# qiyunzhu/woltka

Measured on AMD Instinct MI355X. Metric: alignment records/sec classified, higher is better.
Workload: dtype u8; 1 GPU; synthetic SAM text of 50M reads x <=16 hits (10.50 GB) resident in HBM, 2M-node taxonomy, ranks phylum,genus,species: device tokenizer per 64 MB block + one weighted histogram per sample (the kernels of `woltka classify`, host link left out); records_per_gpu=250034804, reads_per_gpu=50000000

## Files before the change

woltka_amd/csrc/wk_dtok_fused.hpp:

```cpp
#pragma once
#include "wk_dtok.hpp"
#include "wk_dtok_neighbour.hpp"
#include "wk_dtok_planes.hpp"
#include "wk_dtok_rounds.hpp"

namespace wk {

constexpr uint32_t kFzThreads = 512;
constexpr uint32_t kFzWaves = kFzThreads / kWave;
constexpr uint32_t kFzTile = 16384;
constexpr uint32_t kFzBack = 1024;
constexpr uint32_t kFzFwd = 3072;
constexpr uint32_t kFzWin = kFzTile + kFzBack + kFzFwd;
constexpr uint32_t kFzChunks = kFzWin / 16 + 1;
constexpr uint32_t kFzRounds = kFrMaxRounds;
static_assert(kFrChunks * 16u == kFzWin && kFrTailChunk + 1u == kFzChunks && kFrWaves == kFzWaves && kFrWave == kWave,
              "the dealing covers the window");
constexpr uint32_t kFzLines = 1024;
constexpr uint32_t kFzStreams = 4;
constexpr uint32_t kFzCap = 1024;
static_assert(kFzCap >= kFzLines, "a window's records fit an empty buffer");
static_assert(kFzWin + 32 < 65536, "window offsets fit 16 bits");
constexpr uint32_t kFzCarry = 256;
static_assert(kFzCarry + kFzLines <= kFpMaxLines && kFzThreads % kWave == 0, "a window's owned lines fit the planes, a wave's lines one word");

constexpr uint32_t kDtokSpill = 64;

struct FusedArgs {
    const unsigned char* text;
    uint32_t n;
    uint32_t open_end;
    uint32_t span;
    const struct DictSlot8* dict8;
    const uint4* names16;
    uint32_t dict_mask;
    const unsigned char* arena;
    uint2* unknown;
    uint32_t unknown_cap;
    DtokState* state;
    DtokState* host_state;
    const unsigned long long* backup_prev;
    unsigned long long* backup_next;
    uint32_t* host_seq;
    uint32_t seq;
    StreamSet streams;
    const int32_t* submap;
    uint32_t n_submap;
    uint32_t ablate;
};

static_assert(sizeof(DtokState) % 8 == 0, "the packed totals are aligned");
__device__ __forceinline__ unsigned long long* fz_totals(DtokState* state) { return reinterpret_cast<unsigned long long*>(state + 1); }

__global__ void dtok_fused_begin_kernel(unsigned long long* __restrict__ backup, const unsigned long long* __restrict__ cursor, DtokState* state) {
    if (threadIdx.x < (uint32_t)kMaxStreams) backup[threadIdx.x] = cursor[threadIdx.x];
    if (threadIdx.x == 0) {
        *state = DtokState{0u, 0u, 0ull, 0ull, 0ull, 0u, 0u};
        *fz_totals(state) = 0ull;
    }
}

template <int kCtrl, int kRowMask>
__device__ __forceinline__ uint32_t fz_dpp_add(uint32_t v) {
    return v + (uint32_t)__builtin_amdgcn_update_dpp(0, (int)v, kCtrl, kRowMask, 0xF, false);
}
__device__ __forceinline__ uint32_t fz_wave_scan(uint32_t v) {
    static_assert(kWave == 64, "four rows of sixteen lanes");
    v = fz_dpp_add<0x111, 0xF>(v);
    v = fz_dpp_add<0x112, 0xF>(v);
    v = fz_dpp_add<0x114, 0xF>(v);
    v = fz_dpp_add<0x118, 0xF>(v);
    v = fz_dpp_add<0x142, 0xA>(v);
    v = fz_dpp_add<0x143, 0xC>(v);
    return v;
}
__device__ __forceinline__ uint32_t fz_last_lane(uint32_t v) { return (uint32_t)__builtin_amdgcn_readlane((int)v, kWave - 1); }
__device__ __forceinline__ uint32_t fz_wave_sum(uint32_t v) { return fz_last_lane(fz_wave_scan(v)); }
__device__ __forceinline__ unsigned long long fz_first_lane64(unsigned long long v) {
    return ((unsigned long long)(uint32_t)__builtin_amdgcn_readfirstlane((int)(uint32_t)(v >> 32)) << 32) |
           (uint32_t)__builtin_amdgcn_readfirstlane((int)(uint32_t)v);
}

__device__ __forceinline__ uint4 fz_load_stream(const unsigned char* p) {
    typedef uint32_t u32x4 __attribute__((ext_vector_type(4)));
    const u32x4 v = __builtin_nontemporal_load(reinterpret_cast<const u32x4*>(p));
    return make_uint4(v.x, v.y, v.z, v.w);
}
__device__ __forceinline__ unsigned long long fz_load64(const unsigned char* p) {
    unsigned long long w;
    __builtin_memcpy(&w, p, 8);
    return w;
}
__device__ __forceinline__ uint32_t fz_load32(const unsigned char* p) {
    uint32_t w;
    __builtin_memcpy(&w, p, 4);
    return w;
}
__device__ __forceinline__ unsigned long long fz_eq_bytes(unsigned long long w, unsigned char c) {
    const unsigned long long x = w ^ (0x0101010101010101ull * c);
    return ~(((x & 0x7F7F7F7F7F7F7F7Full) + 0x7F7F7F7F7F7F7F7Full) | x | 0x7F7F7F7F7F7F7F7Full);
}
__device__ __forceinline__ uint32_t fz_marks32(uint32_t w, uint32_t c4) {
    const uint32_t x = w ^ c4;
    return ~(((x & 0x7F7F7F7Fu) + 0x7F7F7F7Fu) | x | 0x7F7F7F7Fu);
}
__device__ __forceinline__ unsigned long long fz_low_bytes(unsigned long long w, uint32_t k) {
    return k >= 8u ? w : (w & ((1ull << (8u * k)) - 1ull));
}

__device__ __forceinline__ unsigned long long fz_hash(const unsigned char* p, uint32_t n) {
    unsigned long long h = 0xcbf29ce484222325ull ^ ((unsigned long long)n * 0x9E3779B97F4A7C15ull);
    while (n >= 8u) {
        h = (h ^ fz_load64(p)) * 0x100000001b3ull;
        h ^= h >> 29;
        p += 8;
        n -= 8u;
    }
    const unsigned long long v = n ? fz_low_bytes(fz_load64(p), n) : 0ull;
    h = (h ^ v) * 0x100000001b3ull;
    h ^= h >> 32;
    h *= 0x9E3779B97F4A7C15ull;
    return h ^ (h >> 29);
}

__device__ __forceinline__ bool fz_same(const unsigned char* x, const unsigned char* y, uint32_t n) {
    while (n >= 8u) {
        if (fz_load64(x) != fz_load64(y)) return false;
        x += 8;
        y += 8;
        n -= 8u;
    }
    return n == 0u || fz_low_bytes(fz_load64(x) ^ fz_load64(y), n) == 0ull;
}

struct FzProbe {
    unsigned long long hv, n0, n1;
    uint32_t h;
    uint2 slot;
};
__device__ __forceinline__ FzProbe fz_probe_begin(const FusedArgs& a, const unsigned char* name, uint32_t rn) {
    FzProbe p;
    p.n0 = p.n1 = 0ull;
    if (rn <= 15u) {
        const unsigned long long lo = fz_low_bytes(fz_load64(name), rn), hi = rn > 8u ? fz_low_bytes(fz_load64(name + 8), rn - 8u) : 0ull;
        p.n0 = lo;
        p.n1 = hi | ((unsigned long long)rn << 56);
        unsigned long long h = 0xcbf29ce484222325ull ^ ((unsigned long long)rn * 0x9E3779B97F4A7C15ull), v = lo;
        if (rn >= 8u) {
            h = (h ^ lo) * 0x100000001b3ull;
            h ^= h >> 29;
            v = hi;
        }
        h = (h ^ v) * 0x100000001b3ull;
        h ^= h >> 32;
        h *= 0x9E3779B97F4A7C15ull;
        p.hv = h ^ (h >> 29);
    } else {
        p.hv = fz_hash(name, rn);
    }
    p.h = (uint32_t)p.hv & a.dict_mask;
    p.slot = reinterpret_cast<const uint2*>(a.dict8)[p.h];
    return p;
}
__device__ __forceinline__ int32_t fz_probe_end(const FusedArgs& a, FzProbe p, const unsigned char* name, uint32_t rn, uint32_t abs_off) {
    for (;;) {
        const int32_t id = (int32_t)p.slot.y;
        if (id < 0) break;
        if (p.slot.x == (uint32_t)(p.hv >> 32)) {
            const uint4 nm = a.names16[id];
            const unsigned long long s0 = ((unsigned long long)nm.y << 32) | nm.x, s1 = ((unsigned long long)nm.w << 32) | nm.z;
            if (rn <= 15u) {
                if (s0 == p.n0 && s1 == p.n1) return id;
            } else if ((nm.w >> 24) == 0xFFu) {
                const unsigned char* full = a.arena + nm.x;
                if (fz_load32(full) == rn && fz_same(name, full + 4, rn)) return id;
            }
        }
        p.h = (p.h + 1u) & a.dict_mask;
        p.slot = reinterpret_cast<const uint2*>(a.dict8)[p.h];
    }
    const uint32_t at = atomicAdd(&a.state->n_unknown, 1u);
    if (at < a.unknown_cap)
        a.unknown[at] = make_uint2(abs_off, rn);
    else
        atomicOr(&a.state->flags, kDtokUnknownFull);
    return kLineUnknown;
}

__device__ bool fz_starts_run_slow(const unsigned char* __restrict__ text, uint32_t at, const unsigned char* q, uint32_t qn) {
    uint32_t pos = at;
    while (pos > 0u) {
        const uint32_t e = pos - 1u;
        uint32_t s = e;
        while (s > 0u && text[s - 1u] != '\n') --s;
        uint32_t tab[3], nt = 0;
        for (uint32_t p = s; p < e && nt < 3u; ++p)
            if (text[p] == '\t') tab[nt++] = p;
        if (nt == 3u && !(tab[2] - tab[1] == 2u && text[tab[1] + 1u] == '*')) {
            if (tab[0] - s != qn) return true;
            for (uint32_t k = 0; k < qn; ++k)
                if (text[s + k] != q[k]) return true;
            return false;
        }
        pos = s;
    }
    return true;
}

constexpr uint32_t kFiSubj = (1u << 23) - 1u;
constexpr uint32_t kFiMateShift = 24;
constexpr uint32_t kFiMapped = 1u << 26;
constexpr uint32_t kFiStart = 1u << 27;
constexpr uint32_t kFiUndecided = 1u << 28;
constexpr uint32_t kFiExcl = 1u << 29;
constexpr uint32_t kFiDropped = 1u << 30;
constexpr uint32_t kFiRead = kFiMapped | (3u << kFiMateShift);
constexpr uint32_t kFiKey = kFiRead | kFiSubj;
constexpr uint32_t kFzPad = 8;
constexpr uint32_t kFzEdgeMeta = 4;

__device__ __forceinline__ uint32_t fz_octet(uint32_t z_lo, uint32_t z_hi) { return (((z_lo >> 7) | (z_hi >> 3)) * 0x00204081u >> 21) & 255u; }

__device__ __forceinline__ uint32_t fz_newlines16(uint4 v) {
    return fz_octet(fz_marks32(v.x, 0x0A0A0A0Au), fz_marks32(v.y, 0x0A0A0A0Au)) | (fz_octet(fz_marks32(v.z, 0x0A0A0A0Au), fz_marks32(v.w, 0x0A0A0A0Au)) << 8);
}

__device__ __forceinline__ uint32_t fz_tabs32(const unsigned char* p, unsigned long long* q0 = nullptr, unsigned long long* q1 = nullptr) {
    unsigned long long w[4];
#pragma unroll
    for (uint32_t i = 0; i < 4; ++i) w[i] = fz_load64(p + 8u * i);
    uint32_t m = 0;
#pragma unroll
    for (uint32_t i = 0; i < 4; ++i)
        m |= fz_octet(fz_marks32((uint32_t)w[i], 0x09090909u), fz_marks32((uint32_t)(w[i] >> 32), 0x09090909u)) << (8u * i);
    if (q0) {
        *q0 = w[0];
        *q1 = w[1];
    }
    return m;
}

__global__ void __launch_bounds__(kFzThreads) __attribute__((amdgpu_waves_per_eu(6, 6))) dtok_fused_kernel(FusedArgs a) {
    __shared__ __attribute__((aligned(16))) unsigned char txt[kFzChunks * 16 + 32];
    __shared__ uint16_t ls[kFzLines + 2];
    __shared__ uint16_t f_qn[kFzLines];
    __shared__ __attribute__((aligned(16))) uint32_t edge[kFzLines / kWave + 1][2][8];
    __shared__ __attribute__((aligned(16))) uint32_t info_[kFzPad + kFzCarry + kFzLines + kFzPad + 8];
    __shared__ uint32_t carry[kFzCarry];
    __shared__ unsigned long long planes[kFpPlanes][kFpWords];
    __shared__ uint32_t rbuf[kFzStreams][kFzCap];
    __shared__ unsigned long long fill_packed;
    static_assert(kFzStreams <= 4 && kFzCap + kFzThreads < 65536, "four 16-bit counts");
    __shared__ unsigned long long gbase[kFzStreams];
    __shared__ uint32_t wtot[kFzWaves];
    __shared__ unsigned long long gbase_out[kMaxStreams];
    __shared__ unsigned long long wg_totals;
    __shared__ uint32_t own[4];
    __shared__ uint32_t wg_flags;
    uint32_t* const info = info_ + kFzPad + kFzCarry;

    const uint32_t tid = threadIdx.x, lane = tid & (kWave - 1), wave = tid / kWave;
    const uint32_t wave_s = (uint32_t)__builtin_amdgcn_readfirstlane((int)wave);
    const uint32_t n_streams = a.streams.n_streams;
    const uint32_t ablate = a.ablate;
    const int32_t* const submap = a.submap;
    unsigned long long fill = 0ull;
    if (tid == 0) fill_packed = 0ull;
    if (tid < 4u) reinterpret_cast<uint32_t*>(txt + kFrTailChunk * 16u)[tid] = 0u;
    if (tid == 0) wg_flags = 0u;
    if (tid == 0) wg_totals = 0ull;
    if (tid == 0) edge[0][1][kFzEdgeMeta] = 0u;
    uint32_t my_flags = 0, my_reads = 0, my_lines = 0;
    const uint32_t text_end = a.n + (a.open_end ? 1u : 0u);

    auto flush_all = [&](unsigned long long have, bool last) {
        __syncthreads();
        if (tid < n_streams) {
            const uint32_t cnt = (ablate & 64u) ? 0u : (uint32_t)(have >> (16u * tid)) & 0xFFFFu;
            unsigned long long base = 0ull;
            if (cnt) {
                base = atomicAdd(&a.streams.cursor[tid], (unsigned long long)cnt);
                if (base + cnt > a.streams.cap) atomicOr(&wg_flags, kDtokSpill);
            }
            gbase[tid] = base;
        }
        __syncthreads();
        for (uint32_t k = 0; k < n_streams; ++k) {
            const uint32_t cnt = (ablate & 64u) ? 0u : (uint32_t)(have >> (16u * k)) & 0xFFFFu;
            const unsigned long long base = gbase[k];
            for (uint32_t i = tid; i < cnt; i += kFzThreads)
                if (base + i < a.streams.cap) a.streams.out[k][base + i] = rbuf[k][i];
        }
        if (last) return;
        __syncthreads();
    };

    const uint32_t t0 = blockIdx.x * a.span;
    const uint32_t t1 = a.n - t0 > a.span ? t0 + a.span : a.n;
    const uint32_t span_w1 = (uint32_t)min((unsigned long long)t1 + kFzFwd, (unsigned long long)text_end);
    uint32_t wpos = t0 >= kFzBack ? t0 - kFzBack : 0u;
    uint32_t mode = 0u;
    uint32_t counted = t0;
    bool wide = false;
    uint32_t nc = 0u;
    uint32_t cq_pos = 0u, cq_len = 0u;
    const uint32_t max_trips = a.span / 16u + 2u;
    for (uint32_t trip = 0;; ++trip) {
        if (trip >= max_trips) {
            my_flags |= kDtokSpill;
            break;
        }
        const uint32_t w0 = wpos & ~15u;
        const uint32_t lead = wpos - w0;
        const uint32_t w1 = (uint32_t)min((mode == 0u ? (unsigned long long)t0 + kFzTile + kFzFwd : (unsigned long long)w0 + kFzWin),
                                           (unsigned long long)(wide ? text_end : span_w1));
        const bool to_end = w1 == text_end;
        const bool last_win = wide || w1 == span_w1;
        __syncthreads();
        if (tid < 3u) own[tid] = tid < 2u ? 0xFFFFFFFFu : 0u;
        if (tid < kFzPad) info[-(int32_t)nc - 1 - (int32_t)tid] = kFiStart;
        for (uint32_t i = tid; i < nc; i += kFzThreads) info[(int32_t)i - (int32_t)nc] = carry[i];

        const uint32_t wave_c0 = fr_first_chunk(wave_s), wave_rounds = fr_rounds(wave_s);
        uint4 v[kFzRounds];
#pragma unroll
        for (uint32_t r = 0; r < kFzRounds; ++r) {
            const uint32_t p = w0 + (wave_c0 + r * kWave + lane) * 16u;
            v[r] = make_uint4(0u, 0u, 0u, 0u);
            if (r < wave_rounds && p < a.n && p < w1) v[r] = fz_load_stream(a.text + p);
        }
        uint32_t marks[kFzRounds];
        uint32_t nl_packed = 0;
        bool blank = false;
        const uint32_t in_lo = max(wpos, counted), in_hi = min(min(w1, a.n), t1);
#pragma unroll
        for (uint32_t r = 0; r < kFzRounds; ++r) {
            const uint32_t c = wave_c0 + r * kWave + lane;
            const uint32_t p = w0 + c * 16u;
            marks[r] = 0u;
            if (r >= wave_rounds) continue;
            const uint32_t rp0 = w0 + (wave_c0 + r * kWave) * 16u;
            const bool interior = rp0 >= in_lo && (unsigned long long)rp0 + kWave * 16u <= in_hi;
            *reinterpret_cast<uint4*>(txt + c * 16u) = v[r];
            if (interior) {
                const uint32_t m = fr_chunk_marks(fz_newlines16(v[r]), &blank);
                const uint32_t cnt = (uint32_t)__popc(m);
                my_lines += cnt;
                marks[r] = m;
                nl_packed |= fr_pack(cnt, r);
            } else if (p < w1) {
                uint32_t m = fz_newlines16(v[r]);
                if (p + 16u > a.n) m &= p >= a.n ? 0u : (1u << (a.n - p)) - 1u;
                if (p >= counted && p < t1) my_lines += (uint32_t)__popc(m);
                if (a.open_end && a.n >= p && a.n < p + 16u) m |= 1u << (a.n - p);
                if (p + 16u > w1) m &= (1u << (w1 - p)) - 1u;
                if (p < wpos) m &= ~((1u << (wpos - p)) - 1u);
                m = fr_chunk_marks(m, &blank);
                marks[r] = m;
                nl_packed |= fr_pack((uint32_t)__popc(m), r);
            }
        }
        if (blank && !(ablate & 16u)) my_flags |= kDtokShortLine;
        const uint32_t nl_inc = fz_wave_scan(nl_packed);
        const uint32_t nl_wave = fz_last_lane(nl_inc);
        if (lane == 0) wtot[wave] = fr_total(nl_wave);
        __syncthreads();
        uint32_t before = 0, total_nl = 0;
#pragma unroll
        for (uint32_t w = 0; w < kFzWaves; ++w) {
            before += w < wave ? wtot[w] : 0u;
            total_nl += wtot[w];
        }
        const bool too_many = total_nl + 1u > kFzLines || (ablate & (32u | 512u));
        if (too_many) {
            if (!(ablate & 512u)) my_flags |= kDtokSpill;
        } else {
            if (tid == 0) ls[0] = (uint16_t)lead;
            uint32_t line = before;
#pragma unroll
            for (uint32_t r = 0; r < kFzRounds; ++r) {
                if (r >= wave_rounds) continue;
                const uint32_t c = wave_c0 + r * kWave + lane;
                uint32_t at = line + fr_unpack(nl_inc, r) - (uint32_t)__popc(marks[r]);
                uint32_t m = marks[r];
                while (m) {
                    const uint32_t b = (uint32_t)__ffs((int)m) - 1u;
                    ls[++at] = (uint16_t)(c * 16u + b + 1u);
                    m &= m - 1u;
                }
                line += fr_unpack(nl_wave, r);
            }
        }
        __syncthreads();
        const uint32_t trail = too_many ? wpos : w0 + (uint32_t)__builtin_amdgcn_readfirstlane((int)(uint32_t)ls[total_nl]);
        if (!too_many && last_win && trail >= t0 && trail < t1) my_flags |= kDtokSpill;
        const uint32_t first_line = mode != 0u || w0 == 0u ? 0u : 1u;
        const uint32_t n_lines = too_many ? 0u : total_nl;
        if (tid == 0 && first_line) info[0] = 0u;

        for (uint32_t k0 = first_line; k0 < n_lines; k0 += kFzThreads) {
            const uint32_t k = k0 + tid;
            const bool has = k < n_lines;
            uint32_t word = 0, s = 0, qn = 0, rb = 0, rn = 0;
            unsigned long long q0 = 0ull, q1 = 0ull;
            if (has) {
                s = ls[k];
                const uint32_t e = (uint32_t)ls[k + 1] - 1u;
                uint32_t tab[3] = {0, 0, 0}, nt = 0;
                if (!(ablate & 256u)) {
                    uint32_t m = fz_tabs32(txt + s, &q0, &q1);
                    if (e - s < 32u) m &= (1u << (e - s)) - 1u;
                    nt = min((uint32_t)__popc(m), 3u);
                    tab[0] = s + (uint32_t)__ffs((int)m) - 1u;
                    m &= m - 1u;
                    tab[1] = s + (uint32_t)__ffs((int)m) - 1u;
                    m &= m - 1u;
                    tab[2] = s + (uint32_t)__ffs((int)m) - 1u;
                    for (uint32_t p = s + 32u; nt < 3u && p < e; p += 32u) {
                        m = fz_tabs32(txt + p);
                        if (e - p < 32u) m &= (1u << (e - p)) - 1u;
                        for (; m && nt < 3u; m &= m - 1u) {
                            const uint32_t q = p + (uint32_t)__ffs((int)m) - 1u;
                            if (nt == 0u)
                                tab[0] = q;
                            else if (nt == 1u)
                                tab[1] = q;
                            else
                                tab[2] = q;
                            ++nt;
                        }
                    }
                }
                if (ablate & 16u) {
                } else if (nt < 3u) {
                    my_flags |= kDtokShortLine;
                } else {
                    const uint32_t fl = tab[1] - tab[0] - 1u;
                    const unsigned long long fw = fz_load64(txt + tab[0] + 1u);
                    uint32_t flag = 0;
                    bool digits = fl >= 1u && fl <= 6u;
                    for (uint32_t i = 0; i < fl && i < 6u; ++i) {
                        const uint32_t d = ((uint32_t)(fw >> (8u * i)) & 0xFFu) - (uint32_t)'0';
                        digits &= d <= 9u;
                        flag = flag * 10u + d;
                    }
                    rb = tab[1] + 1u;
                    rn = tab[2] - rb;
                    if (!digits) {
                        my_flags |= kDtokShortLine;
                    } else if (rn == 1u && txt[rb] == '*') {
                    } else {
                        const uint32_t mate = (flag >> 6) & 3u;
                        if (mate == 3u) my_flags |= kDtokBothMates;
                        word = kFiMapped | (mate << kFiMateShift);
                        qn = tab[0] - s;
                        f_qn[k] = (uint16_t)qn;
                    }
                }
            }
            const bool mapped = (word & kFiMapped) != 0u, look = mapped && w0 + s >= t0;
            const unsigned char* const name = txt + rb;
            FzProbe probe;
            if (look && !(ablate & 1u)) probe = fz_probe_begin(a, name, rn);
            const FnLine me = has ? fn_line(mapped, qn, q0, q1) : fn_no_line();
            FnLine prev;
            prev.meta = (uint32_t)__builtin_amdgcn_update_dpp(0, (int)me.meta, 0x138 , 0xF, 0xF, false);
#pragma unroll
            for (uint32_t i = 0; i < 4; ++i) prev.b[i] = (uint32_t)__builtin_amdgcn_update_dpp(0, (int)me.b[i], 0x138, 0xF, 0xF, false);
            const uint32_t verdict = (ablate & 8u) ? (uint32_t)kFnStarts : (uint32_t)fn_verdict(prev, me);
            if (lane == 0 || lane == kWave - 1u) {
                uint32_t* const to = lane == 0 ? edge[(k0 - first_line) / kWave + wave][0] : edge[(k0 - first_line) / kWave + wave + 1u][1];
                *reinterpret_cast<uint4*>(to) = make_uint4(me.b[0], me.b[1], me.b[2], me.b[3]);
                to[kFzEdgeMeta] = me.meta;
            }
            const bool start = look && verdict == kFnStarts;
            if (look) {
                int32_t sid = (ablate & 1u) ? (int32_t)(fz_load32(name + 4) % 1000u) : fz_probe_end(a, probe, name, rn, w0 + rb);
                bool excluded = false;
                if (submap && sid >= 0) {
                    if ((uint32_t)sid < a.n_submap) {
                        sid = submap[sid];
                        if (sid == kLineExcluded) {
                            excluded = true;
                            sid = 0;
                        }
                    } else {
                        my_flags |= kDtokSpill;
                        sid = -1;
                    }
                }
                word |= (start ? kFiStart : 0u) | (verdict == kFnUndecided ? kFiUndecided : 0u) | (excluded ? kFiExcl : 0u) |
                        (sid < 0 ? kFiSubj : ((uint32_t)sid & kFiSubj));
            }
            if (has) info[k] = word;
            const unsigned long long b_all = __ballot(start), b_in = __ballot(start && w0 + s < t1), b_out = b_all & ~b_in;
            if (lane == 0 && b_all) {
                if (b_in) atomicMin(&own[0], k + (uint32_t)__builtin_ctzll(b_in));
                if (b_out) atomicMin(&own[1], k + (uint32_t)__builtin_ctzll(b_out));
                atomicMax(&own[2], k + 63u - (uint32_t)__builtin_clzll(b_all));
            }
        }
        __syncthreads();
        for (uint32_t k0 = first_line; k0 < n_lines; k0 += kFzThreads) {
            const uint32_t k = k0 + tid;
            const uint32_t mk = k < n_lines ? info[k] : 0u;
            bool und = (mk & kFiUndecided) != 0u, start = false;
            if (lane == 0 && und) {
                const uint32_t g = (k0 - first_line) / kWave + wave;
                FnLine before, me;
#pragma unroll
                for (uint32_t i = 0; i < 4; ++i) {
                    before.b[i] = edge[g][1][i];
                    me.b[i] = edge[g][0][i];
                }
                before.meta = edge[g][1][kFzEdgeMeta];
                me.meta = edge[g][0][kFzEdgeMeta];
                const FnVerdict v = fn_verdict(before, me);
                und = v == kFnUndecided;
                start = v == kFnStarts;
                if (g == 0u && nc == 0u && (mode == 1u || wpos == 0u)) {
                    und = false;
                    start = true;
                }
            }
            if (__ballot(und) != 0ull) {
                if (und) {
                    uint32_t j = k;
                    bool found = false;
                    while (j > first_line) {
                        --j;
                        if (info[j] & kFiMapped) {
                            found = true;
                            break;
                        }
                    }
                    if (found)
                        start = f_qn[j] != f_qn[k] || !fz_same(txt + ls[k], txt + ls[j], f_qn[k]);
                    else if (nc)
                        start = f_qn[k] != cq_len || !fz_same(txt + ls[k], a.text + cq_pos, cq_len);
                    else if (mode == 1u || wpos == 0u)
                        start = true;
                    else
                        start = fz_starts_run_slow(a.text, w0 + ls[first_line], txt + ls[k], f_qn[k]);
                }
            }
            if (mk & kFiUndecided) {
                info[k] = (mk & ~kFiUndecided) | (start ? kFiStart : 0u);
                if (start) {
                    atomicMin(&own[w0 + ls[k] < t1 ? 0 : 1], k);
                    atomicMax(&own[2], k);
                }
            }
        }
        __syncthreads();
        const uint32_t o0 = (uint32_t)__builtin_amdgcn_readfirstlane((int)own[0]), o1 = (uint32_t)__builtin_amdgcn_readfirstlane((int)own[1]);
        const uint32_t last = (uint32_t)__builtin_amdgcn_readfirstlane((int)own[2]);
        const uint32_t lpos = w0 + (uint32_t)__builtin_amdgcn_readfirstlane((int)(uint32_t)ls[o0 != 0xFFFFFFFFu ? last : 0u]);
        const bool has_first = nc != 0u || o0 != 0xFFFFFFFFu;
        const int32_t first_own = nc ? -(int32_t)nc : (int32_t)o0;
        int32_t ka = 0, kb = 0;
        uint32_t next = 0u, next_mode = 0u, nc_next = 0u;
        bool more = false, again = false, put_aside = false;
        if (too_many) {
            if ((ablate & (32u | 512u)) && !last_win) {
                next = w1;
                next_mode = 2u;
                more = true;
            }
        } else if (o1 != 0xFFFFFFFFu) {
            kb = (int32_t)o1;
            ka = has_first ? first_own : kb;
        } else if (to_end) {
            kb = (int32_t)n_lines;
            ka = has_first ? first_own : kb;
        } else if (last_win && a.span <= kFzTile) {
            if (o0 != 0xFFFFFFFFu) my_flags |= kDtokSpill;
        } else if (o0 != 0xFFFFFFFFu && (nc != 0u || last != o0 || lpos > wpos)) {
            kb = (int32_t)last;
            ka = first_own;
            next = lpos;
            next_mode = 1u;
            more = true;
            again = last_win;
        } else if (o0 != 0xFFFFFFFFu && last_win && !wide) {
            next = wpos;
            next_mode = 1u;
            more = again = true;
        } else if (o0 != 0xFFFFFFFFu || nc != 0u) {
            put_aside = true;
        } else if (!last_win) {
            next = trail;
            next_mode = 2u;
            more = trail > wpos && trail < t1;
            if (trail <= wpos) my_flags |= kDtokSpill;
        }
        if (put_aside) {
            if (tid == 0) {
                uint32_t c = nc;
                for (uint32_t k = first_line; k < n_lines; ++k) {
                    const uint32_t w = info[k];
                    if (w & kFiMapped) {
                        if (c < kFzCarry) carry[c] = w & ~kFiDropped;
                        ++c;
                    }
                }
                own[3] = c;
            }
            __syncthreads();
            nc_next = (uint32_t)__builtin_amdgcn_readfirstlane((int)own[3]);
            if (nc_next > kFzCarry || trail <= wpos) {
                my_flags |= kDtokSpill;
                nc_next = 0u;
            } else {
                if (nc == 0u) {
                    cq_pos = wpos;
                    cq_len = (uint32_t)__builtin_amdgcn_readfirstlane((int)(uint32_t)f_qn[0]);
                }
                next = trail;
                next_mode = 2u;
                more = true;
                again = last_win;
            }
        }
        for (int32_t k0 = ka; k0 < kb; k0 += (int32_t)kFzThreads) {
            const int32_t k = k0 + (int32_t)tid;
            const uint32_t mk = k < kb ? info[k] : 0u;
            const bool mapped = (mk & kFiMapped) != 0u, excl = mapped && (mk & kFiExcl);
            if (excl) {
                int32_t j = k;
                while (!(info[j] & kFiStart)) --j;
                atomicOr(&info[j], kFiDropped);
            }
            bool dup = false;
            if (mapped && !excl && !(mk & kFiStart) && !(ablate & 2u)) {
                bool done = false;
                for (int32_t j = k; !done; j -= 8) {
                    uint32_t w[8];
#pragma unroll
                    for (uint32_t i = 0; i < 8; ++i) w[i] = info[j - 1 - (int32_t)i];
#pragma unroll
                    for (uint32_t i = 0; i < 8; ++i) {
                        dup |= !done && ((w[i] ^ mk) & kFiKey) == 0u;
                        done |= (w[i] & kFiStart) != 0u;
                    }
                }
            }
            const bool first = mapped && !excl && !dup;
            const uint32_t mate = (mk >> kFiMateShift) & 3u;
            const uint32_t wi = (uint32_t)__builtin_amdgcn_readfirstlane((int)((uint32_t)(k0 - ka) / kWave + wave));
            const bool put = lane == 0 && wi < kFpWords;
            const unsigned long long p_start = __ballot(mapped && (mk & kFiStart));
            if (put) planes[kFpStart][wi] = p_start;
#pragma unroll
            for (uint32_t m = 0; m < 4; ++m) {
                const unsigned long long p_first = __ballot(first && mate == m);
                if (put) planes[kFpFirst + m][wi] = p_first;
            }
        }
        __syncthreads();
        for (int32_t k0 = ka; k0 < kb; k0 += (int32_t)kFzThreads) {
            const int32_t k = k0 + (int32_t)tid;
            bool rec = false;
            uint32_t word = 0, sl = 0, at = 0;
            const uint32_t li = (uint32_t)(k - ka);
            const uint32_t mk = k < kb ? info[k] : 0u;
            const unsigned long long* const mine = planes[kFpFirst + ((mk >> kFiMateShift) & 3u)];
            if (k < kb && ((mine[li / 64u] >> (li % 64u)) & 1ull) && !(ablate & 4u)) {
                uint32_t pos = 0, size = 1;
                bool dropped = (mk & kFiStart) && (mk & kFiDropped);
                if (!(ablate & (2u | 128u))) {
                    const FpRead r = fp_read(planes[kFpStart], mine, li, (uint32_t)(kb - ka));
                    pos = r.pos;
                    size = r.size;
                    dropped = (info[ka + (int32_t)r.head] & kFiDropped) != 0u;
                }
                if (size > (uint32_t)WK_WEIGHT_MAX_K) my_flags |= kDtokBigRead;
                const uint32_t s = mk & kFiSubj;
                if (s != kFiSubj && !dropped) {
                    rec = true;
                    word = s | ((pos & 15u) << kWordSubjBits) | ((size & 31u) << kWordSizeShift);
                    sl = s / kSliceBins;
                    if (sl >= n_streams) sl = n_streams - 1u;
                    my_reads += pos == 0u ? 1u : 0u;
                }
            }
            {
                unsigned long long add = 0;
                uint32_t mine_before = 0;
                for (uint32_t s2 = 0; s2 < n_streams; ++s2) {
                    const unsigned long long m = __ballot(rec && sl == s2);
                    add |= (unsigned long long)__popcll(m) << (16u * s2);
                    if (rec && sl == s2) mine_before = (uint32_t)__popcll(m & ((1ull << lane) - 1ull));
                }
                if (add) {
                    unsigned long long base = 0;
                    if (lane == 0) base = atomicAdd(&fill_packed, add);
                    base = fz_first_lane64(base);
                    at = (uint32_t)(base >> (16u * sl)) & 0xFFFFu;
                    at += mine_before;
                }
            }
            __syncthreads();
            unsigned long long now = fz_first_lane64(fill_packed);
            static_assert(kFzCap + 0x7BFFu == 0x7FFFu && 2u * kFzCap + kFzThreads + 0x7BFFu < 0x10000u, "the full test");
            if ((now + 0x7BFF7BFF7BFF7BFFull) & 0x8000800080008000ull) {
                flush_all(fill, false);
                at -= (uint32_t)(fill >> (16u * sl)) & 0xFFFFu;
                now -= fill;
                if (tid == 0) fill_packed = now;
            }
            if (rec) rbuf[sl][at] = word;
            fill = now;
            if (k0 + (int32_t)kFzThreads < kb) __syncthreads();
        }
        if (!more) break;
        wpos = next;
        mode = next_mode;
        wide = again;
        nc = nc_next;
        counted = w1;
    }
    if (my_flags) atomicOr(&wg_flags, my_flags);
    {
        const uint32_t reads_w = fz_wave_sum(my_reads), lines_w = fz_wave_sum(my_lines);
        const unsigned long long t = ((unsigned long long)lines_w << 32) | reads_w;
        if (lane == 0 && t) atomicAdd(&wg_totals, t);
    }
    flush_all(fill, true);
    __syncthreads();
    if (tid == 0) {
        if (wg_totals) __hip_atomic_fetch_add(fz_totals(a.state), wg_totals, __ATOMIC_RELAXED, __HIP_MEMORY_SCOPE_AGENT);
        if (wg_flags) atomicOr(&a.state->flags, wg_flags);
        __threadfence();
        own[0] = atomicAdd(&a.state->done, 1u) == gridDim.x - 1u ? 1u : 0u;
    }
    __syncthreads();
    if (own[0]) {
        __threadfence();
        uint32_t xt = tid;
        asm volatile("" : "+v"(xt));
        if (xt < (uint32_t)kMaxStreams) {
            const unsigned long long cur = __hip_atomic_load(&a.streams.cursor[xt], __ATOMIC_RELAXED, __HIP_MEMORY_SCOPE_AGENT);
            a.backup_next[xt] = cur;
            gbase_out[xt] = xt < n_streams ? cur - a.backup_prev[xt] : 0ull;
        }
        __syncthreads();
        if (tid == 0) {
            DtokState st{};
            st.flags = __hip_atomic_load(&a.state->flags, __ATOMIC_RELAXED, __HIP_MEMORY_SCOPE_AGENT);
            st.n_unknown = __hip_atomic_load(&a.state->n_unknown, __ATOMIC_RELAXED, __HIP_MEMORY_SCOPE_AGENT);
            const unsigned long long totals = __hip_atomic_load(fz_totals(a.state), __ATOMIC_RELAXED, __HIP_MEMORY_SCOPE_AGENT);
            for (uint32_t k = 0; k < (uint32_t)kMaxStreams; ++k) st.n_out += gbase_out[k];
            st.n_reads = totals & 0xFFFFFFFFull;
            st.n_lines = totals >> 32;
            *a.host_state = st;
            *a.state = DtokState{0u, 0u, 0ull, 0ull, 0ull, 0u, 0u};
            *fz_totals(a.state) = 0ull;
            __threadfence_system();
            if (a.host_seq) __hip_atomic_store(a.host_seq, a.seq, __ATOMIC_RELEASE, __HIP_MEMORY_SCOPE_SYSTEM);
        }
    }
}

}
```

woltka_amd/csrc/wk_dtok_neighbour.hpp:

```cpp
#pragma once
#include <cstdint>

#if defined(__HIPCC__) || defined(__CUDACC__)
#define WK_FN_FN __host__ __device__ __forceinline__
#else
#define WK_FN_FN inline
#endif

namespace wk {

constexpr uint32_t kFnLine = 1u << 16;
constexpr uint32_t kFnMapped = 1u << 17;
constexpr uint32_t kFnQn = 0xFFFFu;
constexpr uint32_t kFnBytes = 16;

struct FnLine {
    uint32_t meta;
    uint32_t b[4];
};

enum FnVerdict : uint32_t { kFnStarts = 0, kFnContinues = 1, kFnUndecided = 2 };

WK_FN_FN unsigned long long fn_low_bytes(unsigned long long w, uint32_t k) { return k >= 8u ? w : (w & ((1ull << (8u * k)) - 1ull)); }

WK_FN_FN FnLine fn_line(bool mapped, uint32_t qn, unsigned long long w0, unsigned long long w1) {
    FnLine l;
    l.meta = kFnLine | (mapped ? kFnMapped : 0u) | (qn & kFnQn);
    const unsigned long long m0 = fn_low_bytes(w0, qn), m1 = qn > 8u ? fn_low_bytes(w1, qn - 8u) : 0ull;
    l.b[0] = (uint32_t)m0;
    l.b[1] = (uint32_t)(m0 >> 32);
    l.b[2] = (uint32_t)m1;
    l.b[3] = (uint32_t)(m1 >> 32);
    return l;
}
WK_FN_FN FnLine fn_no_line() { return FnLine{0u, {0u, 0u, 0u, 0u}}; }

WK_FN_FN FnVerdict fn_verdict(const FnLine& prev, const FnLine& cur) {
    if ((prev.meta & (kFnLine | kFnMapped)) != (kFnLine | kFnMapped)) return kFnUndecided;
    const uint32_t diff = ((prev.meta ^ cur.meta) & kFnQn) | (prev.b[0] ^ cur.b[0]) | (prev.b[1] ^ cur.b[1]) | (prev.b[2] ^ cur.b[2]) | (prev.b[3] ^ cur.b[3]);
    if (diff) return kFnStarts;
    return (cur.meta & kFnQn) <= kFnBytes ? kFnContinues : kFnUndecided;
}

}
```

Baseline: 16.23 billion records/s.

## Deal lines with a witness lane per wave to drop edge shared-memory pass

The line pass now gives each wave 63 owned lines plus one witness lane that re-parses the previous line, so the DPP neighbour comparison covers wave boundaries without the edge array in shared memory. The second pass that resolved undecided lines is skipped entirely unless some wave saw an undecided verdict, tracked with a shared flag. This removes LDS traffic and a resolution sweep in the common case. The cost is about 1/64 redundant parsing work and more loop trips per window.

```diff
diff --git a/woltka_amd/csrc/wk_dtok_fused.hpp b/woltka_amd/csrc/wk_dtok_fused.hpp
--- a/woltka_amd/csrc/wk_dtok_fused.hpp
+++ b/woltka_amd/csrc/wk_dtok_fused.hpp
@@ -217,7 +217,7 @@
 constexpr uint32_t kFiRead = kFiMapped | (3u << kFiMateShift);
 constexpr uint32_t kFiKey = kFiRead | kFiSubj;
 constexpr uint32_t kFzPad = 8;
-constexpr uint32_t kFzEdgeMeta = 4;
+static_assert(kFwWave == kWave && kFwWaves == kFzWaves, "the line pass's dealing is this workgroup's");
 
 __device__ __forceinline__ uint32_t fz_octet(uint32_t z_lo, uint32_t z_hi) { return (((z_lo >> 7) | (z_hi >> 3)) * 0x00204081u >> 21) & 255u; }
 
@@ -244,7 +244,6 @@
     __shared__ __attribute__((aligned(16))) unsigned char txt[kFzChunks * 16 + 32];
     __shared__ uint16_t ls[kFzLines + 2];
     __shared__ uint16_t f_qn[kFzLines];
-    __shared__ __attribute__((aligned(16))) uint32_t edge[kFzLines / kWave + 1][2][8];
     __shared__ __attribute__((aligned(16))) uint32_t info_[kFzPad + kFzCarry + kFzLines + kFzPad + 8];
     __shared__ uint32_t carry[kFzCarry];
     __shared__ unsigned long long planes[kFpPlanes][kFpWords];
@@ -255,7 +254,7 @@
     __shared__ uint32_t wtot[kFzWaves];
     __shared__ unsigned long long gbase_out[kMaxStreams];
     __shared__ unsigned long long wg_totals;
-    __shared__ uint32_t own[4];
+    __shared__ uint32_t own[5];
     __shared__ uint32_t wg_flags;
     uint32_t* const info = info_ + kFzPad + kFzCarry;
 
@@ -269,7 +268,6 @@
     if (tid < 4u) reinterpret_cast<uint32_t*>(txt + kFrTailChunk * 16u)[tid] = 0u;
     if (tid == 0) wg_flags = 0u;
     if (tid == 0) wg_totals = 0ull;
-    if (tid == 0) edge[0][1][kFzEdgeMeta] = 0u;
     uint32_t my_flags = 0, my_reads = 0, my_lines = 0;
     const uint32_t text_end = a.n + (a.open_end ? 1u : 0u);
 
@@ -317,7 +315,7 @@
         const bool to_end = w1 == text_end;
         const bool last_win = wide || w1 == span_w1;
         __syncthreads();
-        if (tid < 3u) own[tid] = tid < 2u ? 0xFFFFFFFFu : 0u;
+        if (tid < 5u) own[tid] = tid < 2u ? 0xFFFFFFFFu : 0u;
         if (tid < kFzPad) info[-(int32_t)nc - 1 - (int32_t)tid] = kFiStart;
         for (uint32_t i = tid; i < nc; i += kFzThreads) info[(int32_t)i - (int32_t)nc] = carry[i];
 
@@ -398,9 +396,10 @@
         const uint32_t n_lines = too_many ? 0u : total_nl;
         if (tid == 0 && first_line) info[0] = 0u;
 
-        for (uint32_t k0 = first_line; k0 < n_lines; k0 += kFzThreads) {
-            const uint32_t k = k0 + tid;
-            const bool has = k < n_lines;
+        const bool first_starts = nc == 0u && (mode == 1u || wpos == 0u);
+        for (uint32_t k0 = first_line; k0 < n_lines; k0 += kFwTrip) {
+            const uint32_t k = fw_line(k0, wave, lane);
+            const bool has = fw_has(k, first_line, n_lines), owner = !fw_witness(lane);
             uint32_t word = 0, s = 0, qn = 0, rb = 0, rn = 0;
             unsigned long long q0 = 0ull, q1 = 0ull;
             if (has) {
@@ -454,11 +453,11 @@
                         if (mate == 3u) my_flags |= kDtokBothMates;
                         word = kFiMapped | (mate << kFiMateShift);
                         qn = tab[0] - s;
-                        f_qn[k] = (uint16_t)qn;
+                        if (owner) f_qn[k] = (uint16_t)qn;
                     }
                 }
             }
-            const bool mapped = (word & kFiMapped) != 0u, look = mapped && w0 + s >= t0;
+            const bool mapped = (word & kFiMapped) != 0u, look = owner && mapped && w0 + s >= t0;
             const unsigned char* const name = txt + rb;
             FzProbe probe;
             if (look && !(ablate & 1u)) probe = fz_probe_begin(a, name, rn);
@@ -467,13 +466,10 @@
             prev.meta = (uint32_t)__builtin_amdgcn_update_dpp(0, (int)me.meta, 0x138 , 0xF, 0xF, false);
 #pragma unroll
             for (uint32_t i = 0; i < 4; ++i) prev.b[i] = (uint32_t)__builtin_amdgcn_update_dpp(0, (int)me.b[i], 0x138, 0xF, 0xF, false);
-            const uint32_t verdict = (ablate & 8u) ? (uint32_t)kFnStarts : (uint32_t)fn_verdict(prev, me);
-            if (lane == 0 || lane == kWave - 1u) {
-                uint32_t* const to = lane == 0 ? edge[(k0 - first_line) / kWave + wave][0] : edge[(k0 - first_line) / kWave + wave + 1u][1];
-                *reinterpret_cast<uint4*>(to) = make_uint4(me.b[0], me.b[1], me.b[2], me.b[3]);
-                to[kFzEdgeMeta] = me.meta;
-            }
+            const uint32_t verdict = ((ablate & 8u) || (first_starts && k == first_line)) ? (uint32_t)kFnStarts : (uint32_t)fn_verdict(prev, me);
             const bool start = look && verdict == kFnStarts;
+            const unsigned long long b_und = __ballot(look && verdict == kFnUndecided);
+            if (lane == 0 && b_und != 0ull) own[4] = 1u;
             if (look) {
                 int32_t sid = (ablate & 1u) ? (int32_t)(fz_load32(name + 4) % 1000u) : fz_probe_end(a, probe, name, rn, w0 + rb);
                 bool excluded = false;
@@ -492,7 +488,7 @@
                 word |= (start ? kFiStart : 0u) | (verdict == kFnUndecided ? kFiUndecided : 0u) | (excluded ? kFiExcl : 0u) |
                         (sid < 0 ? kFiSubj : ((uint32_t)sid & kFiSubj));
             }
-            if (has) info[k] = word;
+            if (has && owner) info[k] = word;
             const unsigned long long b_all = __ballot(start), b_in = __ballot(start && w0 + s < t1), b_out = b_all & ~b_in;
             if (lane == 0 && b_all) {
                 if (b_in) atomicMin(&own[0], k + (uint32_t)__builtin_ctzll(b_in));
@@ -501,28 +497,12 @@
             }
         }
         __syncthreads();
+        if (__builtin_amdgcn_readfirstlane((int)own[4])) {
         for (uint32_t k0 = first_line; k0 < n_lines; k0 += kFzThreads) {
             const uint32_t k = k0 + tid;
             const uint32_t mk = k < n_lines ? info[k] : 0u;
-            bool und = (mk & kFiUndecided) != 0u, start = false;
-            if (lane == 0 && und) {
-                const uint32_t g = (k0 - first_line) / kWave + wave;
-                FnLine before, me;
-#pragma unroll
-                for (uint32_t i = 0; i < 4; ++i) {
-                    before.b[i] = edge[g][1][i];
-                    me.b[i] = edge[g][0][i];
-                }
-                before.meta = edge[g][1][kFzEdgeMeta];
-                me.meta = edge[g][0][kFzEdgeMeta];
-                const FnVerdict v = fn_verdict(before, me);
-                und = v == kFnUndecided;
-                start = v == kFnStarts;
-                if (g == 0u && nc == 0u && (mode == 1u || wpos == 0u)) {
-                    und = false;
-                    start = true;
-                }
-            }
+            const bool und = (mk & kFiUndecided) != 0u;
+            bool start = false;
             if (__ballot(und) != 0ull) {
                 if (und) {
                     uint32_t j = k;
@@ -553,6 +533,7 @@
             }
         }
         __syncthreads();
+        }
         const uint32_t o0 = (uint32_t)__builtin_amdgcn_readfirstlane((int)own[0]), o1 = (uint32_t)__builtin_amdgcn_readfirstlane((int)own[1]);
         const uint32_t last = (uint32_t)__builtin_amdgcn_readfirstlane((int)own[2]);
         const uint32_t lpos = w0 + (uint32_t)__builtin_amdgcn_readfirstlane((int)(uint32_t)ls[o0 != 0xFFFFFFFFu ? last : 0u]);
diff --git a/woltka_amd/csrc/wk_dtok_neighbour.hpp b/woltka_amd/csrc/wk_dtok_neighbour.hpp
--- a/woltka_amd/csrc/wk_dtok_neighbour.hpp
+++ b/woltka_amd/csrc/wk_dtok_neighbour.hpp
@@ -42,4 +42,13 @@
     return (cur.meta & kFnQn) <= kFnBytes ? kFnContinues : kFnUndecided;
 }
 
+constexpr uint32_t kFwWave = 64;
+constexpr uint32_t kFwWaves = 8;
+constexpr uint32_t kFwOwners = kFwWave - 1u;
+constexpr uint32_t kFwTrip = kFwWaves * kFwOwners;
+
+WK_FN_FN uint32_t fw_line(uint32_t k0, uint32_t wave, uint32_t lane) { return k0 + kFwOwners * wave + lane - 1u; }
+WK_FN_FN bool fw_witness(uint32_t lane) { return lane == 0u; }
+WK_FN_FN bool fw_has(uint32_t k, uint32_t first_line, uint32_t n_lines) { return k + 1u > first_line && k < n_lines; }
+
 }
```

Measured after the change: 16.72 billion records/s, median of 6. +3.0%, better.
